# uber/aresdb

Measured on AMD Instinct MI355X. Metric: rows/sec, 1B-row filter -> group-by-agg (whole job), higher is better.
Workload: dtype u32 keys / f64 sums; 1 GPU; C3: filter d1<90 -> dims [floor(ts,3600), d1, d2, d3] (4 x uint32) -> SUM(m float32 -> float64) via HashReduce, validity bitmaps with 1% nulls, shard resident in HBM; rows_per_gpu=1000000000, batch_rows=67108864, batches=15, streams_per_query=2, parallelism=1 shard(s), one per GPU

## Files before the change

### aresdb_amd/csrc/algo/transform.hip

```cpp
#include <hip/hip_runtime.h>

#include <dlfcn.h>

#include <algorithm>
#include <map>
#include <memory>
#include <mutex>
#include <string>
#include <vector>

#include "ares_extensions.h"

#include "binding.hpp"
#include "common.hpp"
#include "device_model.hpp"
#include "dim_layout.hpp"
#include "fast_eval.hpp"
#include "hash_reduce_lds.hpp"
#include "lookback.hpp"
#include "sort_reduce_fused.hpp"

#include "transform_kernels.hpp"

namespace ares {
// ... 653 lines not shown
bool pending_fill_tail(int device, const void *base, int width, int length, int *prev, uint64_t *pattern) {
  if (!defer_available() || length <= 0) return false;
  DeferLock lock(device);
  const uint8_t *b = static_cast<const uint8_t *>(base), *end = b + static_cast<size_t>(width) * length;
  auto it = t_state->fills.lower_bound(const_cast<uint8_t *>(b));
  if (it == t_state->fills.end() || it->second.unit != width || it->second.sortIdx) return false;
  if (it->first >= end || it->first + it->second.bytes != end || static_cast<size_t>(it->first - b) % static_cast<size_t>(width)) return false;
  *prev = static_cast<int>(static_cast<size_t>(it->first - b) / static_cast<size_t>(width));
  *pattern = it->second.pattern;
  return true;
}

void retire_fills_for_write(int device, const void *ptr, size_t bytes) {
  if (!ptr || bytes == 0 || !defer_available()) return;
  DeferLock lock(device);
  if (t_state->fills.empty()) return;
  retire_fills(range_of(ptr, bytes), false);
}

void materialize_fills_for_read(int device, const void *ptr, size_t bytes) {
  if (!ptr || bytes == 0 || !defer_available()) return;
  DeferLock lock(device);
  if (t_state->fills.empty()) return;
  const ByteRange r = range_of(ptr, bytes);
  materialize_fills(&r);
}

bool virtual_iota_peek(int device, const uint32_t *indexVector, int n, bool consume) {
  if (!defer_available()) return false;
  DeferLock lock(device);
  PendingIota *io = lazy_iota(indexVector, n);
  if (io && consume) io->consumed = true;
  return io != nullptr;
}

void settle_dimension_vector(int device, const DimensionVector &v, bool rowsOnly) {
  if (!defer_available()) return;
  const size_t cap = v.VectorCapacity > 0 ? static_cast<size_t>(v.VectorCapacity) : 0;
  const size_t rowBytes = dim_row_bytes(v.NumDimsPerDimWidth);
  materialize_fills_for_read(device, v.DimValues, rowBytes * cap);
  if (rowsOnly) return;
  materialize_fills_for_read(device, v.HashValues, 8 * cap);
  materialize_fills_for_read(device, v.IndexVector, 4 * cap);
  materialize_index_vector(device, v.IndexVector);
}

void materialize_index_vector(int device, const uint32_t *indexVector) {
  if (!indexVector || !defer_available()) return;
  DeferLock lock(device);
  auto it = t_state->iotas.find(const_cast<uint32_t *>(indexVector));
  if (it != t_state->iotas.end() && it->second.consumed) write_iota(it);
}

static void flush_deferred_impl(int device, const ByteRange *limboA, const ByteRange *limboB, const uint32_t *exempt = nullptr) {
  if (limboA) grouped_materialize_for_read(device, limboA->lo, static_cast<size_t>(limboA->hi - limboA->lo));
  if (limboB) grouped_materialize_for_read(device, limboB->lo, static_cast<size_t>(limboB->hi - limboB->lo));
  DeferLock lock(device);
  poll_error_words();
  if (limboA) materialize_fills(limboA);
  if (limboB) materialize_fills(limboB);
  for (auto it = t_state->iotas.begin(); it != t_state->iotas.end();) {
    const ByteRange v = range_of(it->first, 4ull * it->second.n);
    const bool wanted = !it->second.consumed || (limboA && v.overlaps(*limboA)) || (limboB && v.overlaps(*limboB));
    it = wanted ? write_iota(it) : std::next(it);
  }
  auto dormant = [&](const uint32_t *idx) {
    bool skipped = false, queued = false;
    for (auto &kv : t_state->limbo) skipped = skipped || kv.second.idx == idx;
    for (auto &kv : t_state->pending) queued = queued || (kv.second.jobs.count && kv.second.idx == idx);
    return skipped && !queued;
  };
  for (;;) {
    auto c = t_state->compactions.begin();
    while (c != t_state->compactions.end() && (c->first == exempt || dormant(c->first))) ++c;
    if (c == t_state->compactions.end()) break;
    run_compaction(c->first);
  }
  ReleaseSet released;
  for (auto &kv : t_state->pending) {
    if (kv.second.overWait && kv.second.jobs.count) released.add(kv.first);
    launch_queue(kv.first, kv.second);
  }
  if (limboA) materialize_limbo(limboA, &released);
  if (limboB) materialize_limbo(limboB, &released);
  released.run(device);
}

void flush_deferred(int device) { flush_deferred_impl(device, nullptr, nullptr); }

void flush_deferred_for_vector(int device, const DimensionVector &v, const void *values, size_t valueBytes) {
  const size_t rowBytes = dim_row_bytes(v.NumDimsPerDimWidth);
  flush_deferred_for_inputs(device, v.DimValues, rowBytes * static_cast<size_t>(v.VectorCapacity > 0 ? v.VectorCapacity : 0),
                            values, valueBytes);
}

void drop_skipped_outputs(int device, const void *a, size_t aBytes, const void *b, size_t bBytes) {
  if (!fuse_available()) return;
  const ByteRange ra = range_of(a, aBytes), rb = range_of(b, bBytes);
  ReleaseSet released;
  {
    DeferLock lock(device);
    for (auto it = t_state->limbo.begin(); it != t_state->limbo.end();) {
      bool hit = false;
      for (const ByteRange &w : it->second.writes) hit = hit || w.overlaps(ra) || w.overlaps(rb);
      it = hit ? drop_limbo(it, &released) : std::next(it);
    }
  }
  released.run(device);
}

void flush_deferred_for_inputs(int device, const void *a, size_t aBytes, const void *b, size_t bBytes) {
  const ByteRange ra = range_of(a, aBytes), rb = range_of(b, bBytes);
  flush_deferred_impl(device, &ra, &rb);
}

static void begin_batch(int device, hipStream_t stream, const uint32_t *indexVector, uint32_t start, int n) {
  if (!fuse_available()) return;
  bool release = false;
  {
    DeferLock lock(device);
    auto lim = t_state->limbo.find(stream);
    if (lim != t_state->limbo.end()) {
      drop_limbo(lim, nullptr);
      release = true;
    }
    t_state->compactions.erase(indexVector);
    t_state->expansions.erase(stream);
    {
      static int calls = 0;
      if ((++calls & 15) == 0) {
        size_t j = 0, jn = 0, c = 0, cn = 0, p = 0, l = 0, e = 0;
        for (auto &kv : t_state->journals) { jn++; j += kv.second.keep.size(); }
// ... 464 lines not shown
                      : (hasIn ? &filter_rows_kernel<false, true> : &filter_rows_kernel<false, false>);
    {
      const int resident = resident_blocks(device, reinterpret_cast<const void *>(kernel), kBlock), cus = compute_units(device);
      const int perUnit = std::max(1, std::min(resident / cus - 1, 6));
      grid = capped_grid(tiles, std::min(kGridCap, cus * perUnit));
    }
    const size_t bitBytes = static_cast<size_t>(tiles) * kBlock * sizeof(uint16_t);
    bits1 = std::make_shared<StreamBuffer>(bitBytes, stream);
    if (two) bits2 = std::make_shared<StreamBuffer>(bitBytes, stream);
    uint32_t *hostPartials = reinterpret_cast<uint32_t *>(pinned_words());
    ARES_LAUNCH("filter_rows_kernel", kernel, grid, kBlock, stream, f, g,
                hasIn ? c.bits->as<uint16_t>() : static_cast<const uint16_t *>(nullptr), bits1->as<uint16_t>(),
                two ? bits2->as<uint16_t>() : static_cast<uint16_t *>(nullptr), c.n0, tiles, hostPartials);
    c.todo.push_back(LazyFilter{f, colRows, pred, n, keep});
    c.bits = bits1;
    c.lastCount = -1;
    generation = ++t_state->filterGeneration;
    c.generation = generation;
  }
  hip_check(hipStreamSynchronize(stream), "hipStreamSynchronize");
  const volatile uint32_t *parts = reinterpret_cast<const volatile uint32_t *>(pinned_words());
  uint32_t count = 0, count2 = 0;
  for (int b = 0; b < grid; b++) {
    count += parts[2 * b];
    count2 += parts[2 * b + 1];
  }
  {
    DeferLock lock(device);
    auto it = t_state->compactions.find(indexVector);
    if (it != t_state->compactions.end() && it->second.generation == generation) {
      it->second.lastCount = static_cast<int>(count);
      if (two) {
        it->second.predicted.valid = true;
        it->second.predicted.g = g;
        it->second.predicted.count = static_cast<int>(count2);
        it->second.predicted.bits = bits2;
      }
    }
    auto j = t_state->journals.find(indexVector);
    if (j != t_state->journals.end() && j->second.valid) j->second.lastCount = static_cast<int>(count);
  }
  return static_cast<int>(count);
}

bool prepare_filter(int device, hipStream_t stream, const EvalParams &p, uint32_t *indexVector, uint8_t *pred, int n,
                    int numForeignTables, const uint32_t *baseCounts, bool *virtualIdx) {
  bool rowSpace = false;
  *virtualIdx = false;
  FastOperands probe;
  if (!is_wide(p.a.kind) && indexVector != nullptr && numForeignTables == 0 && fast_operands(p, probe, true)) {
    *virtualIdx = virtual_iota(device, indexVector, n, true);
    rowSpace = baseCounts == nullptr && row_space_eligible(device, stream, indexVector, n, p.a.length);
  }
  if (rowSpace) flush_deferred_impl(device, nullptr, nullptr, indexVector);
  else flush_deferred(device);
  rowSpace = rowSpace && row_space_eligible(device, stream, indexVector, n, p.a.length);
  if (!rowSpace) mem_note_write(device, pred, static_cast<size_t>(n));
  materialize_index_vector(device, indexVector);
  return rowSpace;
}

int run_filter_two_phase(int device, hipStream_t stream, FastOperands f, uint32_t *indexVector, uint8_t *pred, int n,
                         RecordID **recordIDVectors, int numForeignTables, bool virtualIdx) {
  f.pad = static_cast<int>(reinterpret_cast<uintptr_t>(pred) & 3);
  const int tiles = pred_tiles(n, f.pad);
  const int passes = 1 + numForeignTables;
  constexpr int kPredGridCap = 256 * 16;
  static_assert(kPredGridCap <= kPinnedWords, "the partial counts are read back in one copy");
  const int predGrid = capped_grid(tiles, kPredGridCap);
  auto wsBuf = std::make_shared<StreamBuffer>(CompactSpace::bytes(tiles, passes, predGrid), stream);
  const CompactSpace cs = clear_compact_space(*wsBuf, tiles, passes, predGrid, stream);
  if (virtualIdx) f.idx = nullptr;
  const bool lazy = numForeignTables == 0 && journal_is_valid(device, indexVector);
  uint32_t *partials = cs.extra();
  ARES_LAUNCH("filter_pred_kernel", filter_pred_kernel, predGrid, kBlock, stream, f, pred, cs.tileCounts(), n, tiles,
              lazy ? partials : nullptr);
  if (lazy) {
    uint32_t parts[kPredGridCap];
    read_back_u32(partials, parts, predGrid, stream);
    uint32_t count = 0;
    for (int b = 0; b < predGrid; b++) count += parts[b];
    PendingCompact c;
    c.stream = stream;
    c.idx = indexVector;
    c.pred = pred;
    c.n = n;
    c.pad = f.pad;
    c.virtualIdx = virtualIdx;
    c.ws = wsBuf;
    c.space = cs;
    DeferLock lock(device);
    t_state->compactions[indexVector] = c;
    return static_cast<int>(count);
  }
  mem_note_write(device, indexVector, 4ull * static_cast<size_t>(n));
  for (int t = 0; t < numForeignTables; t++) mem_note_write(device, recordIDVectors[t], 8ull * static_cast<size_t>(n));
  launch_compaction(cs, pred, indexVector, virtualIdx, recordIDVectors, f.pad, n, stream);
  return read_compaction_total(cs, stream);
}

int run_filter_generic(int device, hipStream_t stream, EvalParams p, const ArrayD *arr, uint32_t *indexVector, uint8_t *pred, int n,
                       RecordID **recordIDVectors, int numForeignTables) {
  if (is_wide(p.a.kind)) {
    SinkD s;
    bind_pred_sink(pred, s);
    p.needRow = indexVector != nullptr;
    const int grid = capped_grid((static_cast<int64_t>(n) + kBlock - 1) / kBlock);
    if (arr)
// ... 851 lines not shown
```

### aresdb_amd/csrc/host/abi_library.hpp

```cpp
#pragma once

#include <dlfcn.h>

#include <cstdlib>
#include <cstring>
#include <stdexcept>
#include <string>

#include "ares_driver.h"
#include "ares_extensions.h"
#include "ares_memory.h"

namespace ares_host {

struct AbiError : std::runtime_error {
  explicit AbiError(const std::string &m) : std::runtime_error(m) {}
};

inline intptr_t check(CGoCallResHandle h) {
  if (h.pStrErr) {
    std::string msg(h.pStrErr);
    free(const_cast<char *>(h.pStrErr));
    throw AbiError(msg);
  }
  return reinterpret_cast<intptr_t>(h.res);
}

inline bool declined(CGoCallResHandle h) {
  if (!h.pStrErr || strncmp(h.pStrErr, "not fusable", 11) != 0) return false;
  free(const_cast<char *>(h.pStrErr));
  return true;
}

inline void set_err(char *err, int errLen, const char *msg) {
  if (err && errLen > 0) {
    strncpy(err, msg, static_cast<size_t>(errLen) - 1);
    err[errLen - 1] = 0;
  }
}

struct AbiLibrary {
  void *algoHandle = nullptr, *memHandle = nullptr;
  decltype(&::InitIndexVector) InitIndexVector;
  decltype(&::HashLookup) HashLookup;
  decltype(&::UnaryTransform) UnaryTransform;
  decltype(&::UnaryFilter) UnaryFilter;
  decltype(&::BinaryTransform) BinaryTransform;
  decltype(&::BinaryFilter) BinaryFilter;
  decltype(&::Sort) Sort;
  decltype(&::Reduce) Reduce;
  decltype(&::HashReduce) HashReduce;
  decltype(&::AresFusedFilterHashReduce) FusedFilterHashReduce = nullptr;
  decltype(&::AresFusedFilterSelect) FusedFilterSelect = nullptr;
  decltype(&::AresFusedFilterJoinSelect) FusedFilterJoinSelect = nullptr;
  decltype(&::AresJoinColumnsRun) JoinColumnsRun = nullptr;
  decltype(&::AresJoinColumnBytes) JoinColumnBytes = nullptr;
  decltype(&::AresGeoShapeColumnRun) GeoShapeColumnRun = nullptr;
  decltype(&::AresGeoShapeColumnBytes) GeoShapeColumnBytes = nullptr;
  decltype(&::AresLocalTimeColumnRun) LocalTimeColumnRun = nullptr;
  decltype(&::Expand) Expand;
  decltype(&::DeviceAllocate) DeviceAllocate;
  decltype(&::DeviceFree) DeviceFree;
  decltype(&::WaitForCudaStream) WaitForCudaStream;
  decltype(&::HyperLogLog) HyperLogLog;
  decltype(&::GeoBatchIntersects) GeoBatchIntersects;
  decltype(&::WriteGeoShapeDim) WriteGeoShapeDim;
  decltype(&::AsyncCopyDeviceToDevice) AsyncCopyDeviceToDevice;
  decltype(&::AsyncCopyDeviceToHost) AsyncCopyDeviceToHost;
  decltype(&::AsyncCopyHostToDevice) AsyncCopyHostToDevice;
  decltype(&::HostAlloc) HostAlloc;
  decltype(&::HostFree) HostFree;
  void (*NoteWrite)(int, const void *, size_t) = nullptr;
  void (*NoteActivity)() = nullptr;
  void noteWrite(int device, const void *p, size_t bytes) const {
    if (NoteWrite) NoteWrite(device, p, bytes);
    if (NoteActivity) NoteActivity();
  }

  template <typename F>
  void bind(void *handle, const char *name, F &fn, bool optional = false) {
    fn = reinterpret_cast<F>(dlsym(handle, name));
    if (!fn && !optional) throw AbiError(std::string("missing symbol ") + name);
  }

  AbiLibrary(const char *algoPath, const char *memPath) {
    memHandle = dlopen(memPath, RTLD_NOW | RTLD_LOCAL);
    if (!memHandle) throw AbiError(std::string("dlopen ") + memPath + ": " + dlerror());
    algoHandle = dlopen(algoPath, RTLD_NOW | RTLD_LOCAL);
    if (!algoHandle) throw AbiError(std::string("dlopen ") + algoPath + ": " + dlerror());
    bind(algoHandle, "InitIndexVector", InitIndexVector);
    bind(algoHandle, "HashLookup", HashLookup);
    bind(algoHandle, "UnaryTransform", UnaryTransform);
    bind(algoHandle, "UnaryFilter", UnaryFilter);
    bind(algoHandle, "BinaryTransform", BinaryTransform);
    bind(algoHandle, "BinaryFilter", BinaryFilter);
    bind(algoHandle, "Sort", Sort);
    bind(algoHandle, "Reduce", Reduce);
    bind(algoHandle, "HashReduce", HashReduce);
    bind(algoHandle, "HyperLogLog", HyperLogLog);
    bind(algoHandle, "GeoBatchIntersects", GeoBatchIntersects);
    bind(algoHandle, "WriteGeoShapeDim", WriteGeoShapeDim);
    bind(algoHandle, "Expand", Expand);
    bind(algoHandle, "AresFusedFilterHashReduce", FusedFilterHashReduce, true);
    bind(algoHandle, "AresFusedFilterSelect", FusedFilterSelect, true);
    bind(algoHandle, "AresFusedFilterJoinSelect", FusedFilterJoinSelect, true);
    bind(algoHandle, "AresJoinColumnsRun", JoinColumnsRun, true);
    bind(algoHandle, "AresJoinColumnBytes", JoinColumnBytes, true);
    bind(algoHandle, "AresGeoShapeColumnRun", GeoShapeColumnRun, true);
    bind(algoHandle, "AresGeoShapeColumnBytes", GeoShapeColumnBytes, true);
    bind(algoHandle, "AresLocalTimeColumnRun", LocalTimeColumnRun, true);
    bind(memHandle, "DeviceAllocate", DeviceAllocate);
    bind(memHandle, "DeviceFree", DeviceFree);
    bind(memHandle, "WaitForCudaStream", WaitForCudaStream);
    bind(memHandle, "AsyncCopyDeviceToDevice", AsyncCopyDeviceToDevice);
    bind(memHandle, "AsyncCopyDeviceToHost", AsyncCopyDeviceToHost);
    bind(memHandle, "AsyncCopyHostToDevice", AsyncCopyHostToDevice);
    bind(memHandle, "HostAlloc", HostAlloc);
    bind(memHandle, "HostFree", HostFree);
    bind(memHandle, "AresMemNoteWrite", NoteWrite, true);
    bind(memHandle, "AresMemNoteActivity", NoteActivity, true);
  }
  ~AbiLibrary() {
    if (algoHandle) dlclose(algoHandle);
    if (memHandle) dlclose(memHandle);
  }
};

template <typename T>
struct Pod {
  alignas(T) unsigned char bytes[sizeof(T)];
  Pod() { memset(bytes, 0, sizeof(bytes)); }
  T &operator*() { return *reinterpret_cast<T *>(bytes); }
  T *operator->() { return reinterpret_cast<T *>(bytes); }
  const T &get() const { return *reinterpret_cast<const T *>(bytes); }
};
using IV = Pod<InputVector>;
using OV = Pod<OutputVector>;

}
```

### aresdb_amd/csrc/host/ares_driver.h

```cpp
#ifndef ARES_DRIVER_H_
#define ARES_DRIVER_H_

#include <stdint.h>

#include "ares_algorithm.h"

#ifdef __cplusplus
extern "C" {
#endif

enum AresNodeKind { ARES_NODE_COLUMN = 0, ARES_NODE_CONST_INT = 1, ARES_NODE_CONST_FLOAT = 2, ARES_NODE_UNARY = 3, ARES_NODE_BINARY = 4 };

typedef struct {
  int kind;
  int op;
  int lhs, rhs;
  int table;
  int column;
  int32_t ival;
  float fval;
  int outType;
} AresPlanNode;

typedef struct {
  int joinColumn;
  CuckooHashIndex index;
  int numColumns;
  int numBatches;
  const VectorPartySlice *slices;
  const int *dataTypes;
  int32_t baseBatchID;
  int32_t numRecordsInLastBatch;
} AresForeignTable;

typedef struct {
  const uint8_t *shapeLatLongs;
  int numShapes;
  int totalNumPoints;
  int pointTable;
  int pointColumn;
  int inOrOut;
  int dimIndex;
} AresGeoIntersection;

typedef struct {
  const AresPlanNode *nodes;
  int numNodes;
  const int *filters; int numFilters;
  const int *foreignFilters; int numForeignFilters;
  const int *dimNodes; const int *dimTypes; int numDims;
  int measureNode;
  int aggFunc;
  int measureType;
  int useHashReduction;
  const AresForeignTable *foreignTables; int numForeignTables;
  int useFusedExtension;
  const AresGeoIntersection *geo;
  int isNonAggregation;
  int limit;
  const int16_t *timezoneLookup;
  int timezoneLookupSize;
  const int *convertTzNodes;
  int numConvertTzNodes;
} AresQueryPlan;

typedef struct AresQuery AresQuery;

void *AresDriverOpen(const char *libalgorithmPath, const char *libmemPath, char *err, int errLen);
void AresDriverClose(void *driver);

AresQuery *AresQueryCreate(void *driver, const AresQueryPlan *plan, int device, void *stream, char *err, int errLen);
int AresQueryRunBatch(AresQuery *q, const VectorPartySlice *columns, int numColumns, int size,
                      uint32_t *baseCounts, uint32_t startRow, char *err, int errLen);
int AresQueryRunResidentBatches(AresQuery *q, const VectorPartySlice *columns, int numColumns, const int *sizes, int numBatches,
                                char *err, int errLen);
int AresQueryResultSize(const AresQuery *q);
int AresQueryDone(const AresQuery *q);
void AresQuerySetMaxBatchSize(AresQuery *q, int rows);
int AresQueryResultCapacity(const AresQuery *q);
uint8_t *AresQueryDimensionVector(const AresQuery *q);
uint8_t *AresQueryMeasureVector(const AresQuery *q);
long AresQueryNumCalls(const AresQuery *q);
long AresQueryNumFusedBatches(const AresQuery *q);
int AresQueryFetch(AresQuery *q, uint8_t *dims, uint8_t *measures, char *err, int errLen);
void AresQuerySetLastBatch(AresQuery *q, int isLast);
void AresQuerySetJoinColumns(AresQuery *q, int on);
void AresQuerySetGeoColumn(AresQuery *q, int on);
void AresQuerySetSecondStream(AresQuery *q, void *stream);
void AresQueryAdoptColumns(AresQuery *q, void *const *allocations, int count);
int64_t AresQueryHLLVectorSize(const AresQuery *q);
int AresQueryFetchHLL(AresQuery *q, uint16_t *regCounts, uint8_t *hllVector, char *err, int errLen);
void AresQueryDestroy(AresQuery *q);

typedef int (*AresAllGatherFn)(void *user, const void *send, void *recv, size_t bytesPerRank, void *stream);
typedef struct AresComm AresComm;
AresComm *AresCommCreate(int rank, int nranks, AresAllGatherFn allGather, void *user);
int AresCommRcclUniqueId(uint8_t id[128], char *err, int errLen);
AresComm *AresCommCreateRccl(const uint8_t id[128], int rank, int nranks, int device, char *err, int errLen);
int AresCommCreateLocal(int nranks, int deviceMemory, AresComm **out, char *err, int errLen);
void AresCommDestroy(AresComm *c);
int AresQueryMergeShards(AresQuery *q, AresComm *c, char *err, int errLen);

typedef int (*AresAllToAllFn)(void *user, const void *send, const size_t *sendBytes, const size_t *sendOffsets, void *recv,
                              const size_t *recvBytes, const size_t *recvOffsets, void *stream);
void AresCommSetAllToAll(AresComm *c, AresAllToAllFn allToAll);
int AresQueryMergeShardsPartitioned(AresQuery *q, AresComm *c, int64_t *totalGroups, char *err, int errLen);

typedef struct {
  const void *host;
  size_t bytes;
  VectorPartySlice slice;
  uint64_t cacheKey;
} AresHostColumn;
typedef struct AresColumnCache AresColumnCache;
AresColumnCache *AresColumnCacheCreate(void *driver, int device, size_t budgetBytes);
void AresColumnCacheDestroy(AresColumnCache *c);
int AresQueryRunHostBatches(AresQuery *q, const AresHostColumn *columns, int numColumns, const int *batchSizes,
                            int numBatches, AresColumnCache *cache, uint64_t stats[4], char *err, int errLen);

#ifdef __cplusplus
}
#endif
#endif
```

### aresdb_amd/csrc/host/batch_executor.cpp

```cpp
#include <algorithm>
#include <cstring>

#include "query.hpp"

using namespace ares_host;

void AresQuery::prepareForFiltering(const VectorPartySlice *cols, int ncols, int n, uint32_t *bc, uint32_t start) {
  columns = cols;
  numColumns = ncols;
  size = n;
  batchRows = n;
  baseCounts = bc;
  startRow = start;
  indexVec = alloc<uint32_t>(static_cast<size_t>(n) * 4);
  predVec = alloc<uint8_t>(static_cast<size_t>(n));
}

void AresQuery::prepareForDimAndMeasureEval() {
  if (resultSize + size <= resultCapacity) return;
  const int oldCapacity = resultCapacity;
  resultCapacity = resultSize + size;
  resultCapacity += resultCapacity / 8;
  const int64_t cap = resultCapacity;
  {
// ... 533 lines not shown
    ncols = static_cast<int>(extendedColumns.size());
  }
  if (runBatchFused(cols, ncols, n)) {
    swapStreams();
    return;
  }
  prepareForFiltering(cols, ncols, n, bc, start);
  preExec();
  filter();
  join();
  project();
  reduce();
  postExec();
  swapStreams();
}

extern "C" {

void *AresDriverOpen(const char *libalgorithmPath, const char *libmemPath, char *err, int errLen) {
  try {
    return new AbiLibrary(libalgorithmPath, libmemPath);
  } catch (std::exception &e) {
    set_err(err, errLen, e.what());
    return nullptr;
  }
}

void AresDriverClose(void *driver) { delete static_cast<AbiLibrary *>(driver); }

AresQuery *AresQueryCreate(void *driver, const AresQueryPlan *plan, int device, void *stream, char *err, int errLen) {
  try {
    return new AresQuery(static_cast<AbiLibrary *>(driver), *plan, device, stream);
  } catch (std::exception &e) {
    set_err(err, errLen, e.what());
    return nullptr;
  }
}

int AresQueryRunBatch(AresQuery *q, const VectorPartySlice *columns, int numColumns, int size, uint32_t *baseCounts,
                      uint32_t startRow, char *err, int errLen) {
  try {
    q->runBatch(columns, numColumns, size, baseCounts, startRow);
    return 0;
  } catch (std::exception &e) {
    set_err(err, errLen, e.what());
    try {
      q->cleanupBeforeAggregation();
    } catch (...) {
    }
    return -1;
  }
}

int AresQueryRunResidentBatches(AresQuery *q, const VectorPartySlice *columns, int numColumns, const int *sizes, int numBatches,
                                char *err, int errLen) {
  for (int b = 0; b < numBatches; b++) {
    q->ownedColumns.clear();
    q->isLastBatch = false;
    const int rc = AresQueryRunBatch(q, columns + static_cast<size_t>(b) * numColumns, numColumns, sizes[b], nullptr, 0, err, errLen);
    if (rc != 0) return rc;
  }
  return 0;
}

int AresQueryResultSize(const AresQuery *q) { return q->plan.isNonAggregation ? q->rowsWritten : q->resultSize; }
int AresQueryDone(const AresQuery *q) { return q->done ? 1 : 0; }
void AresQuerySetMaxBatchSize(AresQuery *q, int rows) { q->maxBatchSize = rows > 0 ? rows : 0; }
int AresQueryResultCapacity(const AresQuery *q) { return q->resultCapacity; }
uint8_t *AresQueryDimensionVector(const AresQuery *q) { return q->dimVec[0]; }
uint8_t *AresQueryMeasureVector(const AresQuery *q) { return q->measureVec[0]; }
long AresQueryNumCalls(const AresQuery *q) { return q->calls; }
long AresQueryNumFusedBatches(const AresQuery *q) { return q->fusedBatches; }
void AresQuerySetLastBatch(AresQuery *q, int isLast) { q->isLastBatch = isLast != 0; }
void AresQuerySetSecondStream(AresQuery *q, void *stream) { q->otherStream = stream; }
void AresQueryAdoptColumns(AresQuery *q, void *const *allocations, int count) {
  q->ownedColumns.assign(allocations, allocations + count);
}
int64_t AresQueryHLLVectorSize(const AresQuery *q) { return static_cast<int64_t>(q->hllVectorSize); }

int AresQueryFetchHLL(AresQuery *q, uint16_t *regCounts, uint8_t *hllVector, char *err, int errLen) {
  try {
    const int n = q->resultSize;
    if (n && q->hllDimRegIDCount) q->d2h(regCounts, q->hllDimRegIDCount, static_cast<size_t>(n) * 2);
    if (n && q->hllVector) q->d2h(hllVector, q->hllVector, q->hllVectorSize);
    q->wait();
    return 0;
  } catch (std::exception &e) {
    set_err(err, errLen, e.what());
    return -1;
  }
}

int AresQueryFetch(AresQuery *q, uint8_t *dims, uint8_t *measures, char *err, int errLen) {
  try {
    if (q->plan.isNonAggregation) {
      uint8_t *out = dims;
      for (const std::vector<uint8_t> &v : q->hostSections) out = std::copy(v.begin(), v.end(), out);
      return 0;
    }
    const int n = q->resultSize;
    q->copyDimsD2H(dims, q->dimVec[0], n, n, q->resultCapacity);
    if (n && measures) q->d2h(measures, q->measureVec[0], static_cast<size_t>(n) * q->plan.measureBytes());
    q->wait();
    return 0;
  } catch (std::exception &e) {
    set_err(err, errLen, e.what());
    return -1;
  }
}

void AresQueryDestroy(AresQuery *q) {
  if (!q) return;
  try {
    q->cleanupBeforeAggregation();
    q->releaseAll();
  } catch (...) {
// ... 6 lines not shown
```

### aresdb_amd/csrc/host/query.hpp

```cpp
#pragma once

#include <memory>
#include <utility>
#include <vector>

#include "plan.hpp"

namespace ares_host {

struct RowSpace {
  enum Kind { JOIN_COLUMNS, GEO_COLUMN } kind;
  Plan plan;
  std::vector<std::pair<int, int>> leaves;
  int numAdded = 0;
  struct JoinedTable {
    std::vector<int> columns;
    int first = 0;
  };
  std::vector<JoinedTable> tables;
  struct LocalTime {
    int timeColumn;
    int table;
    int zoneColumn;
    int outType;
// ... 2 lines not shown
    }
  };
  std::vector<LocalTime> localTimes;
  RowSpace(Kind k, const Plan &original) : kind(k), plan(original) {}
};

}

struct AresQuery {
  using Plan = ares_host::Plan;
  using IV = ares_host::IV;

  ares_host::AbiLibrary *lib;
  const Plan plan;
  const Plan *batchPlan = &plan;
  const ares_host::DimLayout layout;
  int device;
  void *stream;
  void *otherStream = nullptr;
  int resultSize = 0, resultCapacity = 0;
  uint8_t *dimVec[2] = {nullptr, nullptr};
  uint8_t *measureVec[2] = {nullptr, nullptr};
  uint8_t *hllVector = nullptr;
  uint16_t *hllDimRegIDCount = nullptr;
  size_t hllVectorSize = 0;
  bool isLastBatch = false;
  uint32_t *geoPredicateVec = nullptr;
  int sizeBeforeGeoFilter = 0;
  std::vector<void *> ownedColumns;
  uint64_t *hashVec[2] = {nullptr, nullptr};
  uint32_t *dimIndexVec[2] = {nullptr, nullptr};
  int size = 0;
  uint32_t *indexVec = nullptr;
  uint8_t *predVec = nullptr;
  uint32_t *baseCounts = nullptr;
  uint32_t startRow = 0;
  const VectorPartySlice *columns = nullptr;
  int numColumns = 0;
  std::vector<uint8_t *> stack;
  std::vector<RecordID *> foreignRids;
  std::vector<std::vector<VectorPartySlice>> foreignSliceArrays;
  long calls = 0, fusedBatches = 0;
  bool fusedDeclined = false;
  std::unique_ptr<ares_host::RowSpace> rowSpace;
  bool rowSpaceDeclined = false;
  std::vector<VectorPartySlice> extendedColumns;
  std::vector<void *> joinedOutputs;
  int maxBatchSize = 0;
  int batchRows = 0;
  int rowsWritten = 0;
  bool done = false;
  std::vector<std::vector<uint8_t>> hostSections;

  AresQuery(ares_host::AbiLibrary *l, const AresQueryPlan &p, int dev, void *s)
      : lib(l), plan(p), layout(plan.dimTypes), device(dev), stream(s) {}

  template <typename T = uint8_t>
  T *alloc(size_t bytes) {
    return reinterpret_cast<T *>(ares_host::check(lib->DeviceAllocate(bytes ? bytes : 1, device)));
  }
  void release(void *p) {
    if (p) ares_host::check(lib->DeviceFree(p, device));
  }
  void wait() { ares_host::check(lib->WaitForCudaStream(stream, device)); }
  void d2d(void *dst, void *src, size_t bytes) {
    if (bytes) ares_host::check(lib->AsyncCopyDeviceToDevice(dst, src, bytes, stream, device));
  }
  void d2h(void *dst, void *src, size_t bytes) { ares_host::check(lib->AsyncCopyDeviceToHost(dst, src, bytes, stream, device)); }
  void copyDimsD2D(uint8_t *to, uint8_t *from, int64_t length, int64_t offset, int64_t toCapacity, int64_t fromCapacity,
                   int64_t fromOffset = 0) {
    ares_host::copy_dimension_vector(layout, to, from, length, offset, toCapacity, fromCapacity,
                                     [this](void *d, void *s, size_t n) { d2d(d, s, n); }, fromOffset);
  }
  void copyDimsD2H(uint8_t *to, uint8_t *from, int64_t length, int64_t toCapacity, int64_t fromCapacity) {
    ares_host::copy_dimension_vector(layout, to, from, length, 0, toCapacity, fromCapacity,
                                     [this](void *d, void *s, size_t n) { d2h(d, s, n); });
  }

  void prepareForFiltering(const VectorPartySlice *cols, int ncols, int n, uint32_t *bc, uint32_t start);
  void prepareForDimAndMeasureEval();
  uint8_t *allocateStackFrame(int dataType, uint32_t *nullsOffset);
  void shrinkStackFrame();
  void releaseInputColumns();
  void cleanupBeforeAggregation();
  void swapResultBuffers();
  void releaseAll();
  DimensionVector dimensionVector(int which) const;

  struct Action {
    enum Kind { NONE, FILTER, MEASURE, DIMENSION } kind = NONE;
    int dimType = 0;
    int64_t valueOff = 0, nullOff = 0;
    int prevResultSize = 0;
  };
  IV columnInput(const AresPlanNode &n, bool withRids = true, bool withTimezone = false);
  void runAction(const Action &a, int functor, IV *in, int arity);
  IV processExpression(int nodeIdx, const Action &action, bool underConvertTz = false);

  void preExec();
  void filter();
  void join();
  void evalDimensions(int prev);
  void project();
  void reduce();
  void postExec() { swapResultBuffers(); }
  void swapStreams() {
    if (otherStream) std::swap(stream, otherStream);
  }
  void runBatch(const VectorPartySlice *cols, int ncols, int n, uint32_t *bc, uint32_t start);

  int recordsNeeded() const { return plan.limit < 0 ? -1 : std::max(plan.limit - rowsWritten, 0); }
  void prepareForDimEval();
  void expandDimensions();
  void projectNonAggr();
  void postExecNonAggr();
  void runBatchNonAggr(const VectorPartySlice *cols, int ncols, int n, uint32_t *bc, uint32_t start);

  bool fusedExpr(int nodeIdx, int outType, AresFusedExpr *e, int *join = nullptr);
  bool fusedFilters(const std::vector<int> &roots, AresFusedExpr *out, int *count, int *joins = nullptr);
  bool fusedDims(AresFusedExpr *out, int *count, int *joins = nullptr);
  bool runBatchFused(const VectorPartySlice *cols, int ncols, int n);
  bool runBatchFusedSelect(const VectorPartySlice *cols, int ncols, int n);

  void setRowSpace(ares_host::RowSpace::Kind kind, bool on);
  int pruningHints(AresFusedExpr *out);
  bool runJoinColumns(ares_host::RowSpace &rs, int n);
  bool runLocalTimeColumns(ares_host::RowSpace &rs, int n);
  bool runGeoColumn(int n);
  bool resolve(const VectorPartySlice *cols, int ncols, int n);
};
```

### aresdb_amd/driver.py

```python
import ctypes as C
import os

import numpy as np

from . import abi
from .executor import DIM_WIDTHS, Binary, Col, Const, QueryPlan, Unary

DRIVER_PATH = os.path.join(abi.LIB_DIR, "libaresdriver.so")

(NODE_COLUMN, NODE_CONST_INT, NODE_CONST_FLOAT, NODE_UNARY, NODE_BINARY) = range(5)


class PlanNode(C.Structure):
    _fields_ = [("kind", C.c_int), ("op", C.c_int), ("lhs", C.c_int), ("rhs", C.c_int), ("table", C.c_int),
                ("column", C.c_int), ("ival", C.c_int32), ("fval", C.c_float), ("outType", C.c_int)]


class ForeignTableC(C.Structure):
    _fields_ = [("joinColumn", C.c_int), ("index", abi.CuckooHashIndex), ("numColumns", C.c_int),
                ("numBatches", C.c_int), ("slices", C.POINTER(abi.VectorPartySlice)), ("dataTypes", C.POINTER(C.c_int)),
                ("baseBatchID", C.c_int32), ("numRecordsInLastBatch", C.c_int32)]


class GeoIntersectionC(C.Structure):
    _fields_ = [("shapeLatLongs", C.c_void_p), ("numShapes", C.c_int), ("totalNumPoints", C.c_int),
                ("pointTable", C.c_int), ("pointColumn", C.c_int), ("inOrOut", C.c_int), ("dimIndex", C.c_int)]


class QueryPlanC(C.Structure):
    _fields_ = [("nodes", C.POINTER(PlanNode)), ("numNodes", C.c_int),
                ("filters", C.POINTER(C.c_int)), ("numFilters", C.c_int),
                ("foreignFilters", C.POINTER(C.c_int)), ("numForeignFilters", C.c_int),
                ("dimNodes", C.POINTER(C.c_int)), ("dimTypes", C.POINTER(C.c_int)), ("numDims", C.c_int),
                ("measureNode", C.c_int), ("aggFunc", C.c_int), ("measureType", C.c_int),
                ("useHashReduction", C.c_int),
                ("foreignTables", C.POINTER(ForeignTableC)), ("numForeignTables", C.c_int),
                ("useFusedExtension", C.c_int), ("geo", C.POINTER(GeoIntersectionC)),
                ("isNonAggregation", C.c_int), ("limit", C.c_int),
                ("timezoneLookup", C.c_void_p), ("timezoneLookupSize", C.c_int),
                ("convertTzNodes", C.POINTER(C.c_int)), ("numConvertTzNodes", C.c_int)]


ALLGATHER_FN = C.CFUNCTYPE(C.c_int, C.c_void_p, C.c_void_p, C.c_void_p, C.c_size_t, C.c_void_p)
ALLTOALL_FN = C.CFUNCTYPE(C.c_int, C.c_void_p, C.c_void_p, C.POINTER(C.c_size_t), C.POINTER(C.c_size_t), C.c_void_p,
                          C.POINTER(C.c_size_t), C.POINTER(C.c_size_t), C.c_void_p)


class HostColumnC(C.Structure):
    _fields_ = [("host", C.c_void_p), ("bytes", C.c_size_t), ("slice", abi.VectorPartySlice), ("cacheKey", C.c_uint64)]


_lib = None


def _driver():
    global _lib
    if _lib is None:
        if not os.path.exists(DRIVER_PATH):
            raise FileNotFoundError(f"{DRIVER_PATH} is missing — build it first "
                                    f"(python -c 'import __graft_entry__ as g; g.build()')")
        lib = C.CDLL(DRIVER_PATH, mode=os.RTLD_NOW | os.RTLD_LOCAL)
        lib.AresDriverOpen.argtypes, lib.AresDriverOpen.restype = [C.c_char_p, C.c_char_p, C.c_char_p, C.c_int], C.c_void_p
        lib.AresDriverClose.argtypes = [C.c_void_p]
        lib.AresQueryCreate.argtypes = [C.c_void_p, C.POINTER(QueryPlanC), C.c_int, C.c_void_p, C.c_char_p, C.c_int]
        lib.AresQueryCreate.restype = C.c_void_p
        lib.AresQueryRunBatch.argtypes = [C.c_void_p, C.POINTER(abi.VectorPartySlice), C.c_int, C.c_int, C.c_void_p,
                                          C.c_uint32, C.c_char_p, C.c_int]
        lib.AresQueryRunBatch.restype = C.c_int
        lib.AresQueryRunResidentBatches.argtypes = [C.c_void_p, C.POINTER(abi.VectorPartySlice), C.c_int, C.POINTER(C.c_int), C.c_int,
                                                    C.c_char_p, C.c_int]
        lib.AresQueryRunResidentBatches.restype = C.c_int
        for name, res in (("AresQueryResultSize", C.c_int), ("AresQueryResultCapacity", C.c_int),
                          ("AresQueryDimensionVector", C.c_void_p), ("AresQueryMeasureVector", C.c_void_p),
                          ("AresQueryNumCalls", C.c_long), ("AresQueryNumFusedBatches", C.c_long),
                          ("AresQueryDone", C.c_int)):
            fn = getattr(lib, name)
            fn.argtypes, fn.restype = [C.c_void_p], res
        lib.AresQueryFetch.argtypes = [C.c_void_p, C.c_void_p, C.c_void_p, C.c_char_p, C.c_int]
        lib.AresQueryFetch.restype = C.c_int
        lib.AresQueryDestroy.argtypes = [C.c_void_p]
        lib.AresQuerySetLastBatch.argtypes = [C.c_void_p, C.c_int]
        lib.AresQuerySetSecondStream.argtypes = [C.c_void_p, C.c_void_p]
        lib.AresQuerySetJoinColumns.argtypes, lib.AresQuerySetJoinColumns.restype = [C.c_void_p, C.c_int], None
        lib.AresQuerySetGeoColumn.argtypes, lib.AresQuerySetGeoColumn.restype = [C.c_void_p, C.c_int], None
        lib.AresQuerySetMaxBatchSize.argtypes, lib.AresQuerySetMaxBatchSize.restype = [C.c_void_p, C.c_int], None
        lib.AresQueryAdoptColumns.argtypes = [C.c_void_p, C.POINTER(C.c_void_p), C.c_int]
        lib.AresCommCreate.argtypes, lib.AresCommCreate.restype = [C.c_int, C.c_int, ALLGATHER_FN, C.c_void_p], C.c_void_p
        lib.AresCommRcclUniqueId.argtypes, lib.AresCommRcclUniqueId.restype = [C.c_void_p, C.c_char_p, C.c_int], C.c_int
        lib.AresCommCreateRccl.argtypes = [C.c_void_p, C.c_int, C.c_int, C.c_int, C.c_char_p, C.c_int]
        lib.AresCommCreateRccl.restype = C.c_void_p
        lib.AresCommDestroy.argtypes = [C.c_void_p]
        lib.AresQueryMergeShards.argtypes, lib.AresQueryMergeShards.restype = [C.c_void_p, C.c_void_p, C.c_char_p, C.c_int], C.c_int
        lib.AresQueryMergeShardsPartitioned.argtypes = [C.c_void_p, C.c_void_p, C.POINTER(C.c_int64), C.c_char_p, C.c_int]
        lib.AresQueryMergeShardsPartitioned.restype = C.c_int
        lib.AresCommSetAllToAll.argtypes, lib.AresCommSetAllToAll.restype = [C.c_void_p, ALLTOALL_FN], None
        lib.AresColumnCacheCreate.argtypes, lib.AresColumnCacheCreate.restype = [C.c_void_p, C.c_int, C.c_size_t], C.c_void_p
        lib.AresColumnCacheDestroy.argtypes = [C.c_void_p]
        lib.AresQueryRunHostBatches.argtypes = [C.c_void_p, C.POINTER(HostColumnC), C.c_int, C.POINTER(C.c_int), C.c_int,
                                                C.c_void_p, C.POINTER(C.c_uint64), C.c_char_p, C.c_int]
        lib.AresQueryRunHostBatches.restype = C.c_int
        lib.AresQueryHLLVectorSize.argtypes, lib.AresQueryHLLVectorSize.restype = [C.c_void_p], C.c_int64
        lib.AresQueryFetchHLL.argtypes = [C.c_void_p, C.c_void_p, C.c_void_p, C.c_char_p, C.c_int]
        lib.AresQueryFetchHLL.restype = C.c_int
        _lib = lib
    return _lib


_handles = {}


def _open(be: abi.Backend):
    key = (be.algorithm_path, be.memory_path)
    if key not in _handles:
        err = C.create_string_buffer(512)
        h = _driver().AresDriverOpen(be.algorithm_path.encode(), be.memory_path.encode(), err, 512)
        if not h:
            raise abi.AresError(err.value.decode())
        _handles[key] = h
    return _handles[key]


class NativeQuery:

    def __init__(self, be: abi.Backend, plan: QueryPlan, column_names, device=0, stream=None,
                 foreign_column_names=None, streams=None):
        if streams:
            stream = streams[0]
        self.be, self.plan, self.device, self.stream = be, plan, device, stream
        self.column_names = list(column_names)
        self.foreign_column_names = foreign_column_names or [sorted(ft.batches) for ft in plan.foreign_tables]
        self._keep = []
        nodes = []
        convert_tz = []

        def emit(e):
            n = PlanNode()
            if isinstance(e, Col):
                n.kind, n.table = NODE_COLUMN, e.table
                n.column = self.column_names.index(e.name) if e.table == 0 else \
                    self.foreign_column_names[e.table - 1].index(e.name)
            elif isinstance(e, Const):
                if isinstance(e.value, float):
                    n.kind, n.fval = NODE_CONST_FLOAT, e.value
                else:
                    n.kind, n.ival = NODE_CONST_INT, int(e.value)
            elif isinstance(e, Unary):
                n.kind, n.op, n.lhs, n.outType = NODE_UNARY, e.op, emit(e.arg), e.out_type
            elif isinstance(e, Binary):
                lhs = emit(e.lhs)
                rhs = emit(e.rhs)
                n.kind, n.op, n.lhs, n.rhs, n.outType = NODE_BINARY, e.op, lhs, rhs, e.out_type
            else:
                raise TypeError(f"unsupported expression node {e!r}")
            nodes.append(n)
            if isinstance(e, Binary) and e.convert_tz:
                convert_tz.append(len(nodes) - 1)
            return len(nodes) - 1

        filters = [emit(f) for f in plan.filters]
        ffilters = [emit(f) for f in plan.foreign_filters]
        dim_nodes = [emit(d.expr) for d in plan.dimensions]
        measure = emit(plan.measure)

        def arr(ctype, values):
            a = (ctype * max(len(values), 1))(*values)
            self._keep.append(a)
            return a

        fts = []
        for ft, names in zip(plan.foreign_tables, self.foreign_column_names):
            nb = len(ft.batches[names[0]])
            slices = arr(abi.VectorPartySlice, [s for name in names for s in ft.batches[name]])
            types = arr(C.c_int, [ft.data_types[name] for name in names])
            f = ForeignTableC()
            f.joinColumn = self.column_names.index(ft.join_column)
            f.index = ft.index
            f.numColumns, f.numBatches = len(names), nb
            f.slices, f.dataTypes = slices, types
            f.baseBatchID, f.numRecordsInLastBatch = ft.base_batch_id, ft.num_records_in_last_batch
            fts.append(f)

        pc = QueryPlanC()
        pc.nodes, pc.numNodes = arr(PlanNode, nodes), len(nodes)
        pc.filters, pc.numFilters = arr(C.c_int, filters), len(filters)
        pc.foreignFilters, pc.numForeignFilters = arr(C.c_int, ffilters), len(ffilters)
        pc.dimNodes, pc.numDims = arr(C.c_int, dim_nodes), len(dim_nodes)
        pc.dimTypes = arr(C.c_int, [d.data_type for d in plan.dimensions])
        pc.measureNode, pc.aggFunc, pc.measureType = measure, plan.agg, plan.measure_type
        pc.useHashReduction = int(plan.use_hash_reduction)
        pc.foreignTables, pc.numForeignTables = arr(ForeignTableC, fts), len(fts)
        pc.useFusedExtension = int(getattr(plan, "use_fused_extension", False))
        pc.isNonAggregation = int(getattr(plan, "is_non_aggregation", False))
        pc.limit = int(getattr(plan, "limit", -1))
        if convert_tz:
            pc.timezoneLookup = getattr(plan, "timezone_lookup", None)
            pc.timezoneLookupSize = int(getattr(plan, "timezone_lookup_size", 0))
            pc.convertTzNodes, pc.numConvertTzNodes = arr(C.c_int, convert_tz), len(convert_tz)
        geo = getattr(plan, "geo", None)
        if geo is not None:
            g = GeoIntersectionC()
            g.shapeLatLongs, g.numShapes, g.totalNumPoints = geo.shape_lat_longs, geo.num_shapes, geo.total_num_points
            g.pointTable, g.inOrOut, g.dimIndex = geo.point_table, int(geo.in_or_out), geo.dim_index
            g.pointColumn = self.column_names.index(geo.point_column) if geo.point_table == 0 else \
                self.foreign_column_names[geo.point_table - 1].index(geo.point_column)
            self._keep.append(g)
            pc.geo = C.pointer(g)
        err = C.create_string_buffer(512)
        self._q = _driver().AresQueryCreate(_open(be), C.byref(pc), device, stream, err, 512)
        if not self._q:
            raise abi.AresError(err.value.decode())
        if streams and len(streams) > 1:
            _driver().AresQuerySetSecondStream(self._q, streams[1])
        self._err = C.create_string_buffer(1024)

    def run(self, columns, size, base_counts=None, start_row=0, is_last_batch=False, owned_allocations=()):
        _driver().AresQuerySetLastBatch(self._q, int(is_last_batch))
        owned = (C.c_void_p * max(len(owned_allocations), 1))(*owned_allocations)
        _driver().AresQueryAdoptColumns(self._q, owned, len(owned_allocations))
        cols = (abi.VectorPartySlice * len(self.column_names))(*[columns[n] for n in self.column_names])
        rc = _driver().AresQueryRunBatch(self._q, cols, len(self.column_names), size, base_counts, start_row,
                                         self._err, 1024)
        if rc != 0:
            raise abi.AresError(self._err.value.decode().strip())

    def pack_batches(self, batches):
        nc = len(self.column_names)
        cols = (abi.VectorPartySlice * (nc * len(batches)))(*[b[0][n] for b in batches for n in self.column_names])
        sizes = (C.c_int * len(batches))(*[int(b[1]) for b in batches])
        return cols, nc, sizes, len(batches)

    def run_batches(self, packed):
        cols, nc, sizes, nb = packed
        rc = _driver().AresQueryRunResidentBatches(self._q, cols, nc, sizes, nb, self._err, 1024)
        if rc != 0:
            raise abi.AresError(self._err.value.decode().strip())

    @property
    def result_size(self):
        return _driver().AresQueryResultSize(self._q)

    @property
    def result_capacity(self):
        return _driver().AresQueryResultCapacity(self._q)

    @property
    def dim_vector(self):
        return _driver().AresQueryDimensionVector(self._q)

    @property
    def measure_vector(self):
        return _driver().AresQueryMeasureVector(self._q)

    @property
    def calls(self):
        return _driver().AresQueryNumCalls(self._q)

    @property
    def fused_batches(self):
        return _driver().AresQueryNumFusedBatches(self._q)

    @property
    def done(self):
        return bool(_driver().AresQueryDone(self._q))

    def set_join_columns(self, on=True):
        _driver().AresQuerySetJoinColumns(self._q, int(bool(on)))

    def set_geo_column(self, on=True):
        _driver().AresQuerySetGeoColumn(self._q, int(bool(on)))

    def set_max_batch_size(self, rows):
        _driver().AresQuerySetMaxBatchSize(self._q, int(rows))

    @property
    def ndw(self):
        return self.plan.num_dims_per_width()

    @property
    def dim_index(self):
        return self.plan.dim_vector_index()

    @property
    def dim_vec(self):
        return [self.dim_vector, 0]

    @property
    def measure_vec(self):
        return [self.measure_vector, 0]

    def call(self, sym, *args):
        return self.be.call(sym, *args)

    def fetch(self):
        plan, n = self.plan, self.result_size
        widths = sorted([d.width for d in plan.dimensions], reverse=True)
        dims_blob = np.empty(max(n * (sum(widths) + len(widths)), 1), np.uint8)
        meas = np.empty(max(n * plan.measure_bytes, 1), np.uint8)
        rc = _driver().AresQueryFetch(self._q, dims_blob.ctypes.data_as(C.c_void_p), meas.ctypes.data_as(C.c_void_p),
                                      self._err, 1024)
        if rc != 0:
            raise abi.AresError(self._err.value.decode().strip())
        order = plan.dim_vector_index()
        starts = np.concatenate([[0], np.cumsum([w * n for w in widths])])
        null_base = int(starts[-1])
        dims, valids = [], []
        for q in range(len(plan.dimensions)):
            d = order[q]
            dims.append(dims_blob[starts[d]:starts[d] + widths[d] * n].copy())
            valids.append(dims_blob[null_base + d * n: null_base + (d + 1) * n].copy())
        return dims, valids, meas[:n * plan.measure_bytes].copy()

    def fetch_hll(self):
# ... 196 lines not shown
```

Before: 91.63 billion rows/s.

## Add look-ahead worker to overlap next batch filter with current reduce

Adds a per-device host worker thread that runs the filter stage of batch b+1 on the alternate stream while the main thread runs join/project/reduce for batch b, then hands the filtered state over. It also scopes deferred flushes during row-space filtering so work queued on other streams that does not touch the filtered column is not forced. The look-ahead path is off by default (kLookAheadDefault=false) unless enabled by env var or API, and it adds threading and state-handoff complexity.

```diff
diff --git a/aresdb_amd/csrc/algo/transform.hip b/aresdb_amd/csrc/algo/transform.hip
--- a/aresdb_amd/csrc/algo/transform.hip
+++ b/aresdb_amd/csrc/algo/transform.hip
@@ -729,7 +729,15 @@
   if (it != t_state->iotas.end() && it->second.consumed) write_iota(it);
 }
 
-static void flush_deferred_impl(int device, const ByteRange *limboA, const ByteRange *limboB, const uint32_t *exempt = nullptr) {
+struct FlushScope {
+  hipStream_t stream;
+  const FastOperands *column;
+  uint32_t colRows;
+  bool outside(hipStream_t owner) const { return owner != stream; }
+  bool reads(const ByteRange &r) const { return column_overlaps(*column, colRows, r); }
+};
+static void flush_deferred_impl(int device, const ByteRange *limboA, const ByteRange *limboB, const uint32_t *exempt = nullptr,
+                                const FlushScope *scope = nullptr) {
   if (limboA) grouped_materialize_for_read(device, limboA->lo, static_cast<size_t>(limboA->hi - limboA->lo));
   if (limboB) grouped_materialize_for_read(device, limboB->lo, static_cast<size_t>(limboB->hi - limboB->lo));
   DeferLock lock(device);
@@ -738,7 +746,8 @@
   if (limboB) materialize_fills(limboB);
   for (auto it = t_state->iotas.begin(); it != t_state->iotas.end();) {
     const ByteRange v = range_of(it->first, 4ull * it->second.n);
-    const bool wanted = !it->second.consumed || (limboA && v.overlaps(*limboA)) || (limboB && v.overlaps(*limboB));
+    bool wanted = !it->second.consumed || (limboA && v.overlaps(*limboA)) || (limboB && v.overlaps(*limboB));
+    if (scope && scope->outside(it->second.stream) && !scope->reads(v)) wanted = false;
     it = wanted ? write_iota(it) : std::next(it);
   }
   auto dormant = [&](const uint32_t *idx) {
@@ -747,14 +756,25 @@
     for (auto &kv : t_state->pending) queued = queued || (kv.second.jobs.count && kv.second.idx == idx);
     return skipped && !queued;
   };
+  auto unrelated = [&](const PendingCompact &c) {
+    if (!scope || !scope->outside(c.stream)) return false;
+    bool hit = false;
+    column_ranges(*scope->column, scope->colRows, [&](const ByteRange &r) { hit = hit || compaction_touches(c, r); });
+    return !hit;
+  };
   for (;;) {
     auto c = t_state->compactions.begin();
-    while (c != t_state->compactions.end() && (c->first == exempt || dormant(c->first))) ++c;
+    while (c != t_state->compactions.end() && (c->first == exempt || dormant(c->first) || unrelated(c->second))) ++c;
     if (c == t_state->compactions.end()) break;
     run_compaction(c->first);
   }
   ReleaseSet released;
   for (auto &kv : t_state->pending) {
+    if (scope && scope->outside(kv.first)) {
+      bool written = false;
+      for (const ByteRange &w : kv.second.writes) written = written || scope->reads(w);
+      if (!written) continue;
+    }
     if (kv.second.overWait && kv.second.jobs.count) released.add(kv.first);
     launch_queue(kv.first, kv.second);
   }
@@ -1325,8 +1345,12 @@
     *virtualIdx = virtual_iota(device, indexVector, n, true);
     rowSpace = baseCounts == nullptr && row_space_eligible(device, stream, indexVector, n, p.a.length);
   }
-  if (rowSpace) flush_deferred_impl(device, nullptr, nullptr, indexVector);
-  else flush_deferred(device);
+  if (rowSpace) {
+    const FlushScope scope{stream, &probe, p.a.length};
+    flush_deferred_impl(device, nullptr, nullptr, indexVector, &scope);
+  } else {
+    flush_deferred(device);
+  }
   rowSpace = rowSpace && row_space_eligible(device, stream, indexVector, n, p.a.length);
   if (!rowSpace) mem_note_write(device, pred, static_cast<size_t>(n));
   materialize_index_vector(device, indexVector);
diff --git a/aresdb_amd/csrc/host/abi_library.hpp b/aresdb_amd/csrc/host/abi_library.hpp
--- a/aresdb_amd/csrc/host/abi_library.hpp
+++ b/aresdb_amd/csrc/host/abi_library.hpp
@@ -2,10 +2,16 @@
 
 #include <dlfcn.h>
 
+#include <condition_variable>
 #include <cstdlib>
 #include <cstring>
+#include <functional>
+#include <map>
+#include <memory>
+#include <mutex>
 #include <stdexcept>
 #include <string>
+#include <thread>
 
 #include "ares_driver.h"
 #include "ares_extensions.h"
@@ -39,8 +45,70 @@
   }
 }
 
+struct LookAheadWorker {
+  std::mutex mu;
+  std::condition_variable cv;
+  std::function<void()> job;
+  bool busy = false, quit = false, claimed = false;
+  std::thread thread;
+
+  bool claim() {
+    std::lock_guard<std::mutex> lock(mu);
+    if (claimed) return false;
+    return claimed = true;
+  }
+  void release() {
+    std::lock_guard<std::mutex> lock(mu);
+    claimed = false;
+  }
+  void submit(std::function<void()> fn) {
+    std::lock_guard<std::mutex> lock(mu);
+    if (!thread.joinable()) thread = std::thread([this] { loop(); });
+    job = std::move(fn);
+    busy = true;
+    cv.notify_all();
+  }
+  void waitIdle() {
+    std::unique_lock<std::mutex> lock(mu);
+    cv.wait(lock, [this] { return !busy; });
+  }
+  void loop() {
+    for (;;) {
+      std::function<void()> fn;
+      {
+        std::unique_lock<std::mutex> lock(mu);
+        cv.wait(lock, [this] { return quit || job; });
+        if (!job) return;
+        fn.swap(job);
+      }
+      fn();
+      {
+        std::lock_guard<std::mutex> lock(mu);
+        busy = false;
+        cv.notify_all();
+      }
+    }
+  }
+  ~LookAheadWorker() {
+    {
+      std::lock_guard<std::mutex> lock(mu);
+      quit = true;
+      cv.notify_all();
+    }
+    if (thread.joinable()) thread.join();
+  }
+};
+
 struct AbiLibrary {
   void *algoHandle = nullptr, *memHandle = nullptr;
+  std::mutex workersMu;
+  std::map<int, std::unique_ptr<LookAheadWorker>> workers;
+  LookAheadWorker &lookAheadWorker(int device) {
+    std::lock_guard<std::mutex> lock(workersMu);
+    std::unique_ptr<LookAheadWorker> &w = workers[device];
+    if (!w) w.reset(new LookAheadWorker);
+    return *w;
+  }
   decltype(&::InitIndexVector) InitIndexVector;
   decltype(&::HashLookup) HashLookup;
   decltype(&::UnaryTransform) UnaryTransform;
@@ -121,6 +189,7 @@
     bind(memHandle, "AresMemNoteActivity", NoteActivity, true);
   }
   ~AbiLibrary() {
+    workers.clear();
     if (algoHandle) dlclose(algoHandle);
     if (memHandle) dlclose(memHandle);
   }
diff --git a/aresdb_amd/csrc/host/ares_driver.h b/aresdb_amd/csrc/host/ares_driver.h
--- a/aresdb_amd/csrc/host/ares_driver.h
+++ b/aresdb_amd/csrc/host/ares_driver.h
@@ -74,6 +74,8 @@
                       uint32_t *baseCounts, uint32_t startRow, char *err, int errLen);
 int AresQueryRunResidentBatches(AresQuery *q, const VectorPartySlice *columns, int numColumns, const int *sizes, int numBatches,
                                 char *err, int errLen);
+void AresQuerySetLookAhead(AresQuery *q, int on);
+long AresQueryNumLookAheadBatches(const AresQuery *q);
 int AresQueryResultSize(const AresQuery *q);
 int AresQueryDone(const AresQuery *q);
 void AresQuerySetMaxBatchSize(AresQuery *q, int rows);
diff --git a/aresdb_amd/csrc/host/batch_executor.cpp b/aresdb_amd/csrc/host/batch_executor.cpp
--- a/aresdb_amd/csrc/host/batch_executor.cpp
+++ b/aresdb_amd/csrc/host/batch_executor.cpp
@@ -609,16 +609,6 @@
   }
 }
 
-int AresQueryRunResidentBatches(AresQuery *q, const VectorPartySlice *columns, int numColumns, const int *sizes, int numBatches,
-                                char *err, int errLen) {
-  for (int b = 0; b < numBatches; b++) {
-    q->ownedColumns.clear();
-    q->isLastBatch = false;
-    const int rc = AresQueryRunBatch(q, columns + static_cast<size_t>(b) * numColumns, numColumns, sizes[b], nullptr, 0, err, errLen);
-    if (rc != 0) return rc;
-  }
-  return 0;
-}
 
 int AresQueryResultSize(const AresQuery *q) { return q->plan.isNonAggregation ? q->rowsWritten : q->resultSize; }
 int AresQueryDone(const AresQuery *q) { return q->done ? 1 : 0; }
diff --git a/aresdb_amd/csrc/host/query.hpp b/aresdb_amd/csrc/host/query.hpp
--- a/aresdb_amd/csrc/host/query.hpp
+++ b/aresdb_amd/csrc/host/query.hpp
@@ -78,7 +78,12 @@
   bool done = false;
   std::vector<std::vector<uint8_t>> hostSections;
 
+  int lookAhead = -1;
+  long lookAheadBatches = 0;
+
   AresQuery(ares_host::AbiLibrary *l, const AresQueryPlan &p, int dev, void *s)
+      : lib(l), plan(p), layout(plan.dimTypes), device(dev), stream(s) {}
+  AresQuery(ares_host::AbiLibrary *l, const Plan &p, int dev, void *s)
       : lib(l), plan(p), layout(plan.dimTypes), device(dev), stream(s) {}
 
   template <typename T = uint8_t>
@@ -135,6 +140,12 @@
   }
   void runBatch(const VectorPartySlice *cols, int ncols, int n, uint32_t *bc, uint32_t start);
 
+  bool lookAheadEligible(int numBatches) const;
+  void runFront(void *onStream, const VectorPartySlice *cols, int ncols, int n);
+  void adoptFront(AresQuery &front);
+  int runResidentLookAhead(ares_host::LookAheadWorker &worker, const VectorPartySlice *cols, int ncols, const int *sizes,
+                           int numBatches, char *err, int errLen);
+
   int recordsNeeded() const { return plan.limit < 0 ? -1 : std::max(plan.limit - rowsWritten, 0); }
   void prepareForDimEval();
   void expandDimensions();
diff --git a/aresdb_amd/csrc/host/resident_batches.cpp b/aresdb_amd/csrc/host/resident_batches.cpp
--- /dev/null
+++ b/aresdb_amd/csrc/host/resident_batches.cpp
@@ -0,0 +1,142 @@
+#include <cstdlib>
+#include <string>
+
+#include "query.hpp"
+
+using namespace ares_host;
+
+namespace {
+int lookahead_override() {
+  static const int v = [] {
+    const char *e = getenv("ARES_DRIVER_LOOKAHEAD");
+    return (e && (e[0] == '0' || e[0] == '1')) ? e[0] - '0' : -1;
+  }();
+  return v;
+}
+constexpr bool kLookAheadDefault = false;
+}
+
+bool AresQuery::lookAheadEligible(int numBatches) const {
+  const int forced = lookahead_override();
+  if (!(forced >= 0 ? forced == 1 : lookAhead >= 0 ? lookAhead == 1 : kLookAheadDefault)) return false;
+  if (plan.isNonAggregation || plan.useFusedExtension) return false;
+  if (!plan.foreign.empty() || !plan.foreignFilters.empty() || plan.hasGeo) return false;
+  if (rowSpace) return false;
+  return otherStream && otherStream != stream && numBatches >= 2;
+}
+
+void AresQuery::runFront(void *onStream, const VectorPartySlice *cols, int ncols, int n) {
+  stream = onStream;
+  prepareForFiltering(cols, ncols, n, nullptr, 0);
+  preExec();
+  filter();
+}
+
+void AresQuery::adoptFront(AresQuery &front) {
+  columns = front.columns;
+  numColumns = front.numColumns;
+  size = front.size;
+  batchRows = front.batchRows;
+  baseCounts = nullptr;
+  startRow = 0;
+  indexVec = front.indexVec;
+  predVec = front.predVec;
+  stack.swap(front.stack);
+  calls += front.calls;
+  front.indexVec = nullptr;
+  front.predVec = nullptr;
+  front.size = 0;
+  front.calls = 0;
+}
+
+int AresQuery::runResidentLookAhead(LookAheadWorker &worker, const VectorPartySlice *cols, int ncols, const int *sizes,
+                                    int numBatches, char *err, int errLen) {
+  AresQuery front(lib, plan, device, nullptr);
+  void *const streams[2] = {stream, otherStream};
+  std::string frontError;
+  auto run_front = [&](int b) {
+    try {
+      front.runFront(streams[b % 2], cols + static_cast<size_t>(b) * ncols, ncols, sizes[b]);
+    } catch (std::exception &e) {
+      frontError = e.what();
+      try {
+        front.cleanupBeforeAggregation();
+      } catch (...) {
+      }
+    }
+  };
+  auto fail = [&](const std::string &what) {
+    set_err(err, errLen, what.c_str());
+    calls += front.calls;
+    try {
+      cleanupBeforeAggregation();
+    } catch (...) {
+    }
+    return -1;
+  };
+  run_front(0);
+  for (int b = 0; b < numBatches; b++) {
+    if (!frontError.empty()) return fail(frontError);
+    ownedColumns.clear();
+    isLastBatch = false;
+    adoptFront(front);
+    const bool ahead = b + 1 < numBatches;
+    if (ahead) {
+      worker.submit([&run_front, b] { run_front(b + 1); });
+      lookAheadBatches++;
+    }
+    try {
+      join();
+      project();
+      reduce();
+      postExec();
+      swapStreams();
+    } catch (std::exception &e) {
+      const std::string what = e.what();
+      if (ahead) {
+        worker.waitIdle();
+        try {
+          front.cleanupBeforeAggregation();
+        } catch (...) {
+        }
+      }
+      return fail(what);
+    }
+    if (ahead) worker.waitIdle();
+  }
+  return 0;
+}
+
+extern "C" {
+
+int AresQueryRunResidentBatches(AresQuery *q, const VectorPartySlice *columns, int numColumns, const int *sizes, int numBatches,
+                                char *err, int errLen) {
+  if (q->lookAheadEligible(numBatches)) {
+    LookAheadWorker &worker = q->lib->lookAheadWorker(q->device);
+    if (worker.claim()) {
+      struct Release {
+        LookAheadWorker &w;
+        ~Release() { w.release(); }
+      } release{worker};
+      try {
+        return q->runResidentLookAhead(worker, columns, numColumns, sizes, numBatches, err, errLen);
+      } catch (std::exception &e) {
+        worker.waitIdle();
+        set_err(err, errLen, e.what());
+        return -1;
+      }
+    }
+  }
+  for (int b = 0; b < numBatches; b++) {
+    q->ownedColumns.clear();
+    q->isLastBatch = false;
+    const int rc = AresQueryRunBatch(q, columns + static_cast<size_t>(b) * numColumns, numColumns, sizes[b], nullptr, 0, err, errLen);
+    if (rc != 0) return rc;
+  }
+  return 0;
+}
+
+void AresQuerySetLookAhead(AresQuery *q, int on) { q->lookAhead = on != 0 ? 1 : 0; }
+long AresQueryNumLookAheadBatches(const AresQuery *q) { return q->lookAheadBatches; }
+
+}
diff --git a/aresdb_amd/driver.py b/aresdb_amd/driver.py
--- a/aresdb_amd/driver.py
+++ b/aresdb_amd/driver.py
@@ -73,7 +73,7 @@
         for name, res in (("AresQueryResultSize", C.c_int), ("AresQueryResultCapacity", C.c_int),
                           ("AresQueryDimensionVector", C.c_void_p), ("AresQueryMeasureVector", C.c_void_p),
                           ("AresQueryNumCalls", C.c_long), ("AresQueryNumFusedBatches", C.c_long),
-                          ("AresQueryDone", C.c_int)):
+                          ("AresQueryDone", C.c_int), ("AresQueryNumLookAheadBatches", C.c_long)):
             fn = getattr(lib, name)
             fn.argtypes, fn.restype = [C.c_void_p], res
         lib.AresQueryFetch.argtypes = [C.c_void_p, C.c_void_p, C.c_void_p, C.c_char_p, C.c_int]
@@ -83,6 +83,7 @@
         lib.AresQuerySetSecondStream.argtypes = [C.c_void_p, C.c_void_p]
         lib.AresQuerySetJoinColumns.argtypes, lib.AresQuerySetJoinColumns.restype = [C.c_void_p, C.c_int], None
         lib.AresQuerySetGeoColumn.argtypes, lib.AresQuerySetGeoColumn.restype = [C.c_void_p, C.c_int], None
+        lib.AresQuerySetLookAhead.argtypes, lib.AresQuerySetLookAhead.restype = [C.c_void_p, C.c_int], None
         lib.AresQuerySetMaxBatchSize.argtypes, lib.AresQuerySetMaxBatchSize.restype = [C.c_void_p, C.c_int], None
         lib.AresQueryAdoptColumns.argtypes = [C.c_void_p, C.POINTER(C.c_void_p), C.c_int]
         lib.AresCommCreate.argtypes, lib.AresCommCreate.restype = [C.c_int, C.c_int, ALLGATHER_FN, C.c_void_p], C.c_void_p
@@ -123,7 +124,7 @@
 class NativeQuery:
 
     def __init__(self, be: abi.Backend, plan: QueryPlan, column_names, device=0, stream=None,
-                 foreign_column_names=None, streams=None):
+                 foreign_column_names=None, streams=None, look_ahead=None):
         if streams:
             stream = streams[0]
         self.be, self.plan, self.device, self.stream = be, plan, device, stream
@@ -211,6 +212,8 @@
             raise abi.AresError(err.value.decode())
         if streams and len(streams) > 1:
             _driver().AresQuerySetSecondStream(self._q, streams[1])
+        if look_ahead is not None:
+            _driver().AresQuerySetLookAhead(self._q, int(bool(look_ahead)))
         self._err = C.create_string_buffer(1024)
 
     def run(self, columns, size, base_counts=None, start_row=0, is_last_batch=False, owned_allocations=()):
@@ -258,6 +261,10 @@
     @property
     def fused_batches(self):
         return _driver().AresQueryNumFusedBatches(self._q)
+
+    @property
+    def look_ahead_batches(self):
+        return _driver().AresQueryNumLookAheadBatches(self._q)
 
     @property
     def done(self):
```

Result: slower. 90.30 billion rows/s (-1.4%).
